# vribeiro1/artspeech

Measured on AMD Instinct MI355X. Metric: articulator-frames/sec (fwd+bwd), higher is better.
Workload: dtype f32

## Files before the change

### artspeech_amd/build.py

```python
import os
import subprocess
import sys

HERE = os.path.dirname(os.path.abspath(__file__))
ROOT = os.path.dirname(HERE)
CSRC = os.path.join(HERE, "csrc")
OBJ = os.path.join(HERE, "csrc", "build")
LIB = os.path.join(HERE, "libartspeech_hip.so")

ARCH = "gfx950"
COMMON = ["-O3", "-fPIC", "-std=c++17", f"-I{os.path.join(ROOT, 'include')}", f"-I{CSRC}"]
SOURCES = {
    "error.cpp": [],
    "prof.hip": [],
    "gemm_f32.hip": [],
    "wgrad_f32.hip": [],
    "lin_f32.hip": [],
    "gemm_s6.hip": [],
    "rowops.hip": [],
    "gru.hip": [],
    "lstm.hip": [],
    "conv.hip": [],
    "scorer_wgrad.hip": [],
    "ctc.hip": [],
    "recog_eval.hip": [],
    "attention.hip": [],
    "metrics.hip": ["-ffp-contract=off"],
    "p2cp_loss.hip": ["-ffp-contract=off"],
    "multi_mlp.hip": [],
    "pca.hip": [],
    "mean_contour.hip": [],
    "pc_eval.hip": ["-ffp-contract=off"],
    "report.hip": ["-ffp-contract=off"],
    "contours.hip": ["-ffp-contract=off"],
    "artspeech.hip": [],
}


def _newer(src, dst, extra=()):
    if not os.path.exists(dst):
        return True
    t = os.path.getmtime(dst)
    return any(os.path.getmtime(s) > t for s in (src, *extra))


def build(force=False, verbose=True):
    hipcc = os.environ.get("HIPCC", "/opt/rocm/bin/hipcc")
    os.makedirs(OBJ, exist_ok=True)
    headers = [os.path.join(CSRC, f) for f in os.listdir(CSRC) if f.endswith(".h")]
    headers.append(os.path.join(ROOT, "include", "artspeech_hip.h"))
    objs, relink = [], force
    for name, extra in SOURCES.items():
        src = os.path.join(CSRC, name)
        obj = os.path.join(OBJ, name.rsplit(".", 1)[0] + ".o")
        objs.append(obj)
        if force or _newer(src, obj, headers):
            cmd = [hipcc, f"--offload-arch={ARCH}", *COMMON, *extra, "-c", src, "-o", obj]
            if name.endswith(".cpp"):
                cmd = [hipcc, *COMMON, "-c", src, "-o", obj]
            if verbose:
                print("[build]", " ".join(cmd), flush=True)
            subprocess.check_call(cmd)
            relink = True
    if relink or not os.path.exists(LIB):
        cmd = [hipcc, f"--offload-arch={ARCH}", "-shared", "-fPIC", "-o", LIB, *objs]
        if verbose:
            print("[build]", " ".join(cmd), flush=True)
        subprocess.check_call(cmd)
    return LIB


if __name__ == "__main__":
    print(build(force="--force" in sys.argv))
```

### artspeech_amd/csrc/artspeech.hip

```cpp
#include <stdlib.h>

#include <algorithm>
#include <mutex>
#include <vector>

#include "as_launch.h"
#include "gemm_internal.h"
#include "rowops.h"

namespace {

constexpr int D = AS_HEAD_HIDDEN;
constexpr int64_t SLAB_FLOATS = 16LL << 20;
constexpr int64_t SLAB2_FLOATS = 28LL << 20;

struct Carve {
    int64_t off = 0;
    int64_t take(int64_t n) {
        const int64_t o = off;
        off += as_round_up(n, 64);
        return o;
    }
};

// ... 212 lines not shown
        lo.Bp = reinterpret_cast<const uint16_t*>(ws + w.w3p); lo.bp_rows = (int)as_round_up(O, OUT_BN);
        lo.bp_batch = as_planes_batch_stride(lo.bp_rows, D); lo.bp_plane = A * lo.bp_batch;
        int n_part = 0;
        if (crit) {
            lo.tgt = crit->tgt; lo.tgt_T = crit->tgt_T; lo.lengths = crit->lengths; lo.T = crit->T; lo.scale = crit->scale;
            lo.dout = crit->dout; lo.partial = ws + w.lpart; lo.partial_capacity = w.lpart_n; lo.loss = crit->loss;
        }
        took = as_lin_out_try(&lo, &n_part, st);
        AS_REQUIRE(took >= 0, took, "head gemm3: launch failed");
        if (took && crit && n_part > 0) AS_TRY(as_loss_final(ws + w.lpart, n_part, crit->scale, crit->loss, st));
        crit_done = took && crit;
        if (!took) {
            took = as_lin_try(&l3, st);
            AS_REQUIRE(took >= 0, took, "head gemm3: launch failed");
        }
    }
    if (!took)
        AS_STEP("head.gemm3", st, gemm_nt(ws + w.r2hat, AD, ws + w.w3f, D, out, (long)A * O, ws + w.b3f, R, O, D, 2, st, A, D,
                       (long)Opad * D, O, O));
    if (crit && !crit_done) {
        AS_STEP("loss", st, as_euclid_masked_fwd_bwd_presigmoid(out, crit->tgt, crit->tgt_T, crit->lengths, (int32_t)(rows / crit->T), crit->T, A,
                                                               d.n_samp, crit->scale, crit->loss, crit->dout, ws + w.lpart, st));
    }
    return 0;
}

int head_bwd_dx(const as_dims& d, const as_layout& L, const float* P, const float* out, const float* dout, int64_t rows,
                float* dx, const float* relu_src, float* ws, hipStream_t st, bool presig = false) {
    (void)L; (void)P;
    const int A = d.n_art, H = d.hidden, O = 2 * d.n_samp;
    const HeadWs w = head_ws(d, rows);
    const int R = (int)rows;
    const long AD = (long)A * D, AO = (long)A * O;
    const float* dpre3 = presig ? dout : ws + w.dpre3;
    if (!presig) AS_STEP("headb.sigmoid", st, as_sigmoid_bwd(out, dout, ws + w.dpre3, rows * AO, st));
    const int Opad = (int)as_round_up(O, 32);
    const unsigned long long* bits1 = reinterpret_cast<const unsigned long long*>(ws + w.bits1);
    const unsigned long long* bits2 = reinterpret_cast<const unsigned long long*>(ws + w.bits2);
    as_lin b3{};
    b3.A = dpre3; b3.lda = AO; b3.a_batch = O;
    b3.B = ws + w.w3f; b3.ldb = D; b3.b_batch = (long)Opad * D; b3.b_kc = 0;
    b3.C = ws + w.dz2; b3.ldc = AD; b3.c_batch = D;
    b3.M = R; b3.N = D; b3.K = Opad; b3.ka_valid = O; b3.batch = A; b3.epi = 2;
    b3.xhat = ws + w.r2hat; b3.ldx = AD; b3.x_batch = D; b3.rstd_in = ws + w.rstd2; b3.bits_in = bits2;
    b3.Bp = reinterpret_cast<const uint16_t*>(ws + w.w3tp); b3.bp_rows = D; b3.bp_batch = as_planes_batch_stride(D, Opad);
    b3.bp_plane = A * b3.bp_batch;
    int took;
    {
        AS_PROF("headb.dx3", st);
        took = as_lin_try(&b3, st);
        AS_REQUIRE(took >= 0, took, "head dx3: launch failed");
    }
    if (!took) {
        AS_STEP("headb.dx3", st, gemm_nn(dpre3, AO, ws + w.w3f, D, ws + w.dz2, AD, R, D, O, st, A, O, (long)Opad * D, D));
        AS_STEP("headb.norm2", st, as_normalize_bwd(ws + w.dz2, ws + w.r2hat, ws + w.rstd2, nullptr, ws + w.dz2, rows * A, D, st, bits2));
    }
    as_lin b2 = b3;
    b2.A = ws + w.dz2; b2.lda = AD; b2.a_batch = D;
    b2.B = ws + w.w2f; b2.b_batch = (long)D * D;
    b2.C = ws + w.dz1; b2.K = D; b2.ka_valid = D;
    b2.xhat = ws + w.r1hat; b2.rstd_in = ws + w.rstd1; b2.bits_in = bits1;
    b2.Bp = reinterpret_cast<const uint16_t*>(ws + w.w2tp); b2.bp_batch = as_planes_batch_stride(D, D); b2.bp_plane = A * b2.bp_batch;
    {
        AS_PROF("headb.dx2", st);
        took = as_lin_try(&b2, st);
        AS_REQUIRE(took >= 0, took, "head dx2: launch failed");
    }
    if (!took) {
        AS_STEP("headb.dx2", st, gemm_nn(ws + w.dz2, AD, ws + w.w2f, D, ws + w.dz1, AD, R, D, D, st, A, D, (long)D * D, D));
        AS_STEP("headb.norm1", st, as_normalize_bwd(ws + w.dz1, ws + w.r1hat, ws + w.rstd1, nullptr, ws + w.dz1, rows * A, D, st, bits1));
    }
    int dx1_slabs = 0;
    if (H <= 256 && H % 4 == 0) {
        as_lin l{};
        l.A = ws + w.dz1; l.lda = AD;
        l.Bp = reinterpret_cast<const uint16_t*>(ws + w.w1tp); l.bp_rows = (int)as_round_up(H, 128);
        l.bp_batch = as_planes_batch_stride(l.bp_rows, (int)AD); l.bp_plane = l.bp_batch;
        l.C = ws + w.slab; l.ldc = H;
        l.M = R; l.N = H; l.K = (int)AD; l.batch = 1;
        const int want = (int)std::max<int64_t>(1, std::min<int64_t>(8, 512 / std::max(1, as_cdiv(R, 64))));
        const int slabs = as_lin_plain_s6_slabs((int)AD, want);
        if ((int64_t)slabs * R * H <= SLAB_FLOATS) {
            AS_PROF("headb.dx1", st);
            const int took1 = as_lin_plain_s6(&l, want, (long)R * H, st);
            AS_REQUIRE(took1 >= 0, took1, "head dx1: launch failed");
            if (took1) dx1_slabs = slabs;
        }
    }
    if (!dx1_slabs)
        AS_STEP("headb.dx1", st, gemm_nn(ws + w.dz1, AD, ws + w.w1f, H, ws + w.dxhat, H, R, H, (int)AD, st, 1, 0, 0, 0, ws + w.slab));
    AS_STEP("headb.norm0", st, as_normalize_bwd(dx1_slabs ? ws + w.slab : ws + w.dxhat, ws + w.xhat, ws + w.rstd0, relu_src, dx, rows, H, st, nullptr,
                                                 dx1_slabs ? dx1_slabs : 1, (long)R * H));
    return 0;
}

struct TrunkJob { const float* dz; const float* y; float* dW; float* db; int H; };

int head_bwd_dw(const as_dims& d, const as_layout& L, const float* P, int64_t rows, float* G, float* ws, float* slab,
                hipStream_t st, const float* dpre3_in = nullptr, int cu_budget = 0, long slab_floats = SLAB_FLOATS,
                const TrunkJob* trunk = nullptr, int part = 0, int unfold_layers = -1) {
    const int A = d.n_art, H = d.hidden, O = 2 * d.n_samp;
    const HeadWs w = head_ws(d, rows);
    const int R = (int)rows;
    const long AD = (long)A * D, AO = (long)A * O;
    const float* dpre3 = dpre3_in ? dpre3_in : ws + w.dpre3;
    as_wgrad_job jobs[4] = {};
    as_gemm& g3 = jobs[0].g;
    g3.A = dpre3; g3.a_i = 1; g3.a_k = AO; g3.a_batch = O; g3.M = O;
    g3.B = ws + w.r2hat; g3.b_j = 1; g3.b_k = AD; g3.b_batch = D; g3.N = D;
    g3.C = ws + w.dw3f; g3.ldc = D; g3.c_batch = (long)O * D; g3.K = R; g3.batch = A;
    g3.colsum = G + L.b3; g3.colsum_batch = O;
    as_gemm& g1 = jobs[1].g;
    g1 = g3;
    g1.A = ws + w.xhat; g1.a_k = H; g1.a_batch = 0; g1.M = H;
    g1.B = ws + w.dz1;
    g1.C = ws + w.dw1f; g1.ldc = H; g1.c_batch = (long)D * H;
    g1.colsum = nullptr; g1.colsum_batch = 0;
    jobs[1].colsum_b = G + L.b1; jobs[1].colsum_b_batch = D; jobs[1].c_trans = 1;
    as_wgrad_job job2{};
    as_gemm& g2 = job2.g;
    g2 = g3;
    g2.A = ws + w.dz2; g2.a_k = AD; g2.a_batch = D; g2.M = D;
    g2.B = ws + w.r1hat;
    g2.C = ws + w.dw2f; g2.c_batch = (long)D * D;
    g2.colsum = G + L.b2; g2.colsum_batch = D;
    const bool multi_ok = R % 32 == 0 && R >= 512;
    if (part == 0 || part == 1) {
        int n = 2;
        const bool trunk_rides = trunk && 2 * trunk->H == 256;
        if (trunk_rides) {
            as_gemm& gt = jobs[n].g;
            gt.A = trunk->dz; gt.a_i = 1; gt.a_k = trunk->H; gt.M = trunk->H;
            gt.B = trunk->y; gt.b_j = 1; gt.b_k = 2 * trunk->H; gt.N = 2 * trunk->H;
            gt.C = trunk->dW; gt.ldc = 2 * trunk->H; gt.K = R; gt.batch = 1;
            gt.colsum = trunk->db; gt.colsum_batch = 0;
            ++n;
        }
        if (part == 0) jobs[n++] = job2;
        int took = 0;
        if (multi_ok) {
            AS_PROF(part == 0 ? "headb.dw_fused" : "headb.dw31", st);
            took = as_wgrad_multi(jobs, n, slab, slab_floats, cu_budget, st, cu_budget > 0);
            AS_REQUIRE(took >= 0, took, "head weight gradients: launch failed");
        }
        if (!took) {
            AS_STEP("headb.dw3", st, gemm_tn(dpre3, AO, ws + w.r2hat, AD, ws + w.dw3f, D, O, D, R, st, slab, G + L.b3, O, A, O, D, (long)O * D, 0, 0, 0, cu_budget));
            AS_STEP("headb.dw1", st, gemm_tn(ws + w.dz1, AD, ws + w.xhat, H, ws + w.dw1f, H, (int)AD, H, R, st, slab, G + L.b1, 0, 1, 0, 0, 0, 0, 0, 0, cu_budget));
            if (part == 0)
                AS_STEP("headb.dw2", st, gemm_tn(ws + w.dz2, AD, ws + w.r1hat, AD, ws + w.dw2f, D, D, D, R, st, slab, G + L.b2, D, A, D, D, (long)D * D, 0, 0, 0, cu_budget));
        }
        if (trunk && !(took && trunk_rides))
            AS_STEP("trunkb.dw", st, gemm_tn(trunk->dz, trunk->H, trunk->y, 2 * trunk->H, trunk->dW, 2 * trunk->H, trunk->H, 2 * trunk->H, R, st, slab, trunk->db, 0));
    } else {
        int took = 0;
        if (multi_ok) {
            AS_PROF("headb.dw2", st);
            took = as_wgrad_multi(&job2, 1, slab, slab_floats, cu_budget, st, cu_budget > 0);
            AS_REQUIRE(took >= 0, took, "head weight gradients: launch failed");
        }
        if (!took)
            AS_STEP("headb.dw2", st, gemm_tn(ws + w.dz2, AD, ws + w.r1hat, AD, ws + w.dw2f, D, D, D, R, st, slab, G + L.b2, D, A, D, D, (long)D * D, 0, 0, 0, cu_budget));
    }
    if (unfold_layers < 0) unfold_layers = part == 1 ? 0 : 7;
    if (unfold_layers == 0) return 0;
    const float* dWf[3]; const float* dbf[3]; const float* Wp[3]; const float* gm[3]; const float* bt[3];
    float* dWo[3]; float* dgm[3]; float* dbt[3];
    int Rs[3], Ks[3], cnt = 0;
// ... 379 lines not shown
```

### artspeech_amd/csrc/gemm_internal.h

```cpp
#pragma once
#include "as_common.h"

int as_wgrad_try(const as_gemm* g, hipStream_t st);
struct as_wgrad_job {
    as_gemm g;
    float* colsum_b; long colsum_b_batch;
    int c_trans;
};
int as_wgrad_multi(const as_wgrad_job* jobs, int n, float* slab, long slab_floats, int cu_budget, hipStream_t st, bool exact = false);

enum { AS_ARITH_FP32 = 0, AS_ARITH_BF16X6 = 1 };
int as_matrix_arith();

struct as_planes_job {
    const float* B; long n_stride, k_stride, batch_stride;
    int batch, N, K, rows_pad, Kpad;
    uint16_t* out;
};
int as_emit_planes(const as_planes_job* jobs, int n, hipStream_t st);
static inline long as_planes_batch_stride(int rows_pad, int Kpad) { return (long)(Kpad / 16) * rows_pad * 16; }
static inline long as_planes_floats(int batch, int rows_pad, int Kpad) { return 3 * batch * as_planes_batch_stride(rows_pad, Kpad) / 2; }

int as_gemm_s6_nt(const float* A, long lda, long a_batch, const float* B, long ldb, long b_batch, const float* bias, long bias_batch, float* C,
                  long ldc, long c_batch, int M, int N, int K, int batch, int act, hipStream_t st);
int as_gemm_s6_nt_ext(const as_gemm* g, hipStream_t st);
template <int N> struct IC2 { static constexpr int value = N; };

void as_stop_event_set_raw(void* ev);
void* as_stop_event_take_raw();
inline void as_stop_event_set(hipEvent_t ev) { as_stop_event_set_raw((void*)ev); }
inline hipEvent_t as_stop_event_take() { return (hipEvent_t)as_stop_event_take_raw(); }

struct as_lin {
    const float* A; long lda, a_batch;
    const float* B; long ldb, b_batch; int b_kc;
    const uint16_t* Bp; long bp_plane, bp_batch; int bp_rows;
    float* C; long ldc, c_batch;
    const float* bias; long bias_batch;
    int M, N, K, ka_valid, batch, act, epi;
    float* rstd; unsigned long long* bits;
    const float* xhat; long ldx, x_batch; const float* rstd_in; const unsigned long long* bits_in;
    int tile_rows;
};
int as_lin_try(const as_lin* a, hipStream_t st);
int as_lin_plain_s6(const as_lin* a, int ksplit, long c_split, hipStream_t st);
static inline int as_lin_plain_s6_slabs(int K, int ksplit) {
    if (ksplit < 1) ksplit = 1;
    const int kchunk = (int)as_round_up(as_cdiv(K, ksplit), 32);
    return as_cdiv(K, kchunk);
}

struct as_lin_out {
    const float* A; long lda, a_batch;
    const float* B; long ldb, b_batch; int b_rows;
    const float* bias; long bias_batch;
    float* out; long ldo, o_batch;
    int M, N, K, batch;
    const float* tgt; long tgt_T; const int* lengths; int T; float scale;
    float* dout; float* partial; long partial_capacity;
    const uint16_t* Bp; long bp_plane, bp_batch; int bp_rows;
    float* loss;
};
int as_lin_out_try(const as_lin_out* a, int* n_partials, hipStream_t st);
int* as_arrival_counter(hipStream_t st);
int as_loss_final(const float* partial, int n, float scale, float* loss, hipStream_t st);

bool as_gru_bwd_tokens_fits(int32_t V, int32_t H, int32_t T);
int as_gru_bidir_bwd_tokens(const float* dy, const float* y, const float* gates, const float* w_hh, const int32_t* lengths,
                            int32_t B, int32_t T, int32_t H, float* dgh, const int64_t* tokens, int64_t tok_stride, int32_t V,
                            float* part, hipStream_t st);
int as_gru_bidir_fwd_tokens(const float* table, const int64_t* tokens, int64_t tok_stride, int32_t V, const float* w_hh,
                            const float* b_hh, const int32_t* lengths, int32_t B, int32_t T, int32_t H, float* y, float* gates,
                            hipStream_t st);
int as_count_bad_tokens(const int64_t* tokens, long tok_stride, int T, long rows, int V, int* count, hipStream_t st);
int as_sum_partials(const float* part, long n, int chunks, float* out, hipStream_t st);
```

### artspeech_amd/csrc/lin_f32.hip

```cpp
#include <cstdlib>

#include <type_traits>

#include "gemm_internal.h"
#include "split_arith.h"

namespace {

constexpr int BN = 256, BK = 16, NT = 512, NBUF = 3;
enum { EPI_PLAIN = 0, EPI_LNF = 1, EPI_LNB = 2 };

struct LinK {
    const float* A; long lda, a_batch;
    const float* B; long ldb, b_batch;
    const uint16_t* Bp; long bp_plane, bp_batch; int bp_rows;
    int kchunk; long c_split;
    float* C; long ldc, c_batch;
    const float* bias; long bias_batch;
    int M, N, K, ka_valid, batch, act;
    int n_big, big_per_batch, big_per_batch_rows, small_per_batch;
    int tile_rows;
    unsigned long long* dbg; long dbg_max;
    float eps;
    float* rstd;
// ... 248 lines not shown
                __builtin_amdgcn_sched_barrier(0);
            }
        }
    };
    static_assert(BK == 16, "two fragment groups per k-tile");
    Frag f0, f1;
    load(f0, 0, 0);
    for (int kt = 0; kt < nk; ++kt) {
        load(f1, kt, 1);
        __builtin_amdgcn_sched_barrier(0);
        mma(f0, kt + AHEADT < nk ? kt + AHEADT : -1);
        __builtin_amdgcn_sched_barrier(0);
        if (kt + 2 < nk) asm volatile("s_waitcnt vmcnt(3)" ::: "memory");
        else asm volatile("s_waitcnt vmcnt(0)" ::: "memory");
        as_wait_lds();
        __builtin_amdgcn_s_barrier();
        if (kt + 1 < nk) load(f0, kt + 1, 0);
        __builtin_amdgcn_sched_barrier(0);
        mma(f1, -1);
        __builtin_amdgcn_sched_barrier(0);
    }
    if (stamp) g.dbg[8L * blockIdx.x + 2] = __builtin_amdgcn_s_memtime();

    lin_epilogue<TM, EPI>(g, acc, smem, bz, m0, tm_eff, wave, lane);
    if (stamp) {
        asm volatile("s_waitcnt vmcnt(0)" ::: "memory");
        g.dbg[8L * blockIdx.x + 3] = __builtin_amdgcn_s_memtime();
        g.dbg[8L * blockIdx.x + 6] = __builtin_amdgcn_s_memrealtime();
    }
}

__device__ __forceinline__ int xcd_contiguous(int b, int total) {
    const int q = total >> 3, r = total & 7, x = b & 7, i = b >> 3;
    return x * q + min(x, r) + i;
}

constexpr int S6_BK = 32;
constexpr int S6_PLANE = 64 * S6_BK * 2;
constexpr int S6_BUF = 3 * S6_PLANE;

template <int N> struct IC { static constexpr int value = N; };

template <int NW, int TME>
__device__ __forceinline__ void s6_main_loop(f32x16 (&acc)[2], unsigned char* sm, const float* __restrict__ A, long lda, int rows_valid,
                                             int K, int ka_valid, const uint16_t* __restrict__ bp, unsigned b_lane, long bp_plane,
                                             long bp_step, int tid, int lane, bool late, unsigned long long* stamp1 = nullptr) {
    constexpr int NTH = NW * 64;
    constexpr int AL = 512 / NTH;
    const int l31 = lane & 31, lh = lane >> 5;
    const int a_chunk = tid & 7;
    unsigned a_off[AL];
    int a_wr[AL];
#pragma unroll
    for (int q = 0; q < AL; ++q) {
        const int row = (tid >> 3) + q * (NTH / 8);
        a_off[q] = (unsigned)(min(row, rows_valid - 1) * (int)lda + a_chunk * 4) * 4u;
        a_wr[q] = row * 64 + (((a_chunk >> 1) ^ ((row >> 2) & 3)) * 16) + (a_chunk & 1) * 8;
    }
    const int nk = K / S6_BK, nj = 2 * nk;
    const gptr Au = as_uniform_ptr(A);
    auto a_load = [&](f32x4 (&dst)[AL], int kt) {
        kt = min(kt, nk - 1);
        const unsigned ko = kt * S6_BK + a_chunk * 4 + 4 <= ka_valid ? (unsigned)(kt * S6_BK) * 4u : 0u - (unsigned)a_chunk * 16u;
#pragma unroll
        for (int q = 0; q < AL; ++q) dst[q] = *reinterpret_cast<gptr_f4>(Au + (a_off[q] + ko));
    };
    auto a_store = [&](const f32x4 (&src)[AL], int buf) {
#pragma unroll
        for (int q = 0; q < AL; ++q) {
            unsigned h0, m0, l0, h1, m1, l1;
            split_pair(src[q].x, src[q].y, h0, m0, l0);
            split_pair(src[q].z, src[q].w, h1, m1, l1);
            unsigned char* d = sm + buf * S6_BUF + a_wr[q];
            *reinterpret_cast<uint2*>(d) = make_uint2(h0, h1);
            *reinterpret_cast<uint2*>(d + S6_PLANE) = make_uint2(m0, m1);
            *reinterpret_cast<uint2*>(d + 2 * S6_PLANE) = make_uint2(l0, l1);
        }
    };
    auto b_load = [&](u32x4 (&dst)[3], int j) {
        j = min(j, nj - 1);
#pragma unroll
        for (int p = 0; p < 3; ++p) dst[p] = *reinterpret_cast<gptr_u4>(as_uniform_ptr(bp + p * bp_plane + j * bp_step) + b_lane);
    };
    const int sw = (l31 >> 2) & 3;
    const unsigned char* a_rd = sm + l31 * 64;

    f32x4 aq[3][AL];
    u32x4 bq[3][3];
    a_load(aq[0], 0);
    a_load(aq[1], 1);
    b_load(bq[0], 0);
    b_load(bq[1], 1);
    a_store(aq[0], 0);
    as_lds_barrier();
    if (stamp1) *stamp1 = __builtin_amdgcn_s_memtime();
    auto tile = [&](auto Uc, int kt) {
        constexpr int U = decltype(Uc)::value;
        const unsigned char* img = a_rd + (kt & 1) * S6_BUF;
        a_load(aq[(U + 2) % 3], kt + 2);
#pragma unroll
        for (int s = 0; s < 2; ++s) {
            b_load(bq[(2 * U + s + 2) % 3], 2 * kt + s + 2);
            __builtin_amdgcn_sched_barrier(0);
            bf16x8 fa[TME][3];
#pragma unroll
            for (int p = 0; p < 3; ++p)
#pragma unroll
                for (int i = 0; i < TME; ++i)
                    fa[i][p] = *reinterpret_cast<const bf16x8*>(img + p * S6_PLANE + i * 32 * 64 + (((2 * s + lh) ^ sw) * 16));
            const u32x4(&bs)[3] = bq[(2 * U + s) % 3];
            bf16x8 fb[3];
#pragma unroll
            for (int p = 0; p < 3; ++p) fb[p] = __builtin_bit_cast(bf16x8, bs[p]);
            constexpr int PA[6] = {0, 0, 0, 1, 1, 2}, PB[6] = {0, 1, 2, 0, 1, 0};
#pragma unroll
            for (int o = 0; o < 6; ++o)
#pragma unroll
                for (int i = 0; i < TME; ++i)
                    acc[i] = __builtin_amdgcn_mfma_f32_32x32x16_bf16(fa[i][PA[o]], fb[PB[o]], acc[i], 0, 0, 0);
            __builtin_amdgcn_sched_barrier(0);
            if (late == (s == 0)) a_store(aq[(U + 1) % 3], (kt & 1) ^ 1);
        }
        as_lds_barrier();
    };
    int kt = 0;
    for (; kt + 3 <= nk; kt += 3) {
        tile(IC<0>{}, kt);
        tile(IC<1>{}, kt + 1);
        tile(IC<2>{}, kt + 2);
    }
    if (kt < nk) tile(IC<0>{}, kt);
    if (kt + 1 < nk) tile(IC<1>{}, kt + 1);
}

template <int EPI>
__global__ __launch_bounds__(NT, 4) void lin_s6_kernel(LinK g) {
    constexpr int EPIT = 32 * BN;
    static_assert(EPIT * 4 >= 2 * S6_BUF, "the epilogue's staging area holds both plane images");
    __shared__ __attribute__((aligned(16))) float smem[EPIT];
    int bz, m0, tm_eff;
    const int tile = blockIdx.x;
    if (tile < g.n_big) {
        bz = tile / g.big_per_batch;
        m0 = (tile - bz * g.big_per_batch) * 64;
        tm_eff = 2;
    } else {
        const int j = tile - g.n_big;
        bz = j / g.small_per_batch;
        m0 = g.big_per_batch_rows + (j - bz * g.small_per_batch) * 32;
        tm_eff = 1;
    }
    const int tid = threadIdx.x, lane = tid & 63, wave = tid >> 6;
    f32x16 acc[2];
#pragma unroll
    for (int i = 0; i < 2; ++i)
#pragma unroll
        for (int r = 0; r < 16; ++r) acc[i][r] = 0.f;
    const uint16_t* bp = g.Bp + (long)bz * g.bp_batch;
    const unsigned b_lane = (unsigned)((wave * 32 + (lane & 31)) * 16 + (lane >> 5) * 8) * 2u;
    unsigned char* sm = reinterpret_cast<unsigned char*>(smem);
    const float* A = g.A + (long)bz * g.a_batch + (long)m0 * g.lda;
    const bool late = __builtin_amdgcn_readfirstlane(wave) >= 4;
    const bool stamp = g.dbg != nullptr && tid == 0 && blockIdx.x < g.dbg_max;
    unsigned long long* d = stamp ? g.dbg + 8L * blockIdx.x : nullptr;
    if (stamp) {
        d[0] = __builtin_amdgcn_s_memtime();
        d[4] = __builtin_amdgcn_s_memrealtime();
        d[5] = __builtin_amdgcn_s_getreg((4 - 1) << 11 | 0 << 6 | 4) | ((unsigned long long)__builtin_amdgcn_s_getreg((32 - 1) << 11 | 0 << 6 | 20) << 32);
    }
    if (tm_eff == 2) s6_main_loop<8, 2>(acc, sm, A, g.lda, g.M - m0, g.K, g.ka_valid, bp, b_lane, g.bp_plane, (long)g.bp_rows * 16, tid, lane, late, stamp ? d + 1 : nullptr);
    else s6_main_loop<8, 1>(acc, sm, A, g.lda, g.M - m0, g.K, g.ka_valid, bp, b_lane, g.bp_plane, (long)g.bp_rows * 16, tid, lane, late, stamp ? d + 1 : nullptr);
    if (stamp) d[2] = __builtin_amdgcn_s_memtime();
    lin_epilogue<2, EPI>(g, acc, smem, bz, m0, tm_eff, wave, lane);
    if (stamp) {
        asm volatile("s_waitcnt vmcnt(0)" ::: "memory");
        d[3] = __builtin_amdgcn_s_memtime();
        d[6] = __builtin_amdgcn_s_memrealtime();
    }
}

template <int NW>
__global__ __launch_bounds__(NW * 64, 4) void lin_s6_plain_kernel(LinK g) {
    __shared__ __attribute__((aligned(16))) unsigned char sm[2 * S6_BUF];
    int bz, m0, tm_eff;
    const int tile = blockIdx.x;
    if (tile < g.n_big) {
        bz = tile / g.big_per_batch;
        m0 = (tile - bz * g.big_per_batch) * 64;
        tm_eff = 2;
    } else {
        const int j = tile - g.n_big;
        bz = j / g.small_per_batch;
        m0 = g.big_per_batch_rows + (j - bz * g.small_per_batch) * 32;
        tm_eff = 1;
    }
    const int tid = threadIdx.x, lane = tid & 63, wave = tid >> 6;
    const int l31 = lane & 31, lh = lane >> 5;
    const int ks = blockIdx.y, k0 = ks * g.kchunk;
    const int klen = min(g.kchunk, g.K - k0);
    const int kav = max(0, min(klen, g.ka_valid - k0));
    f32x16 acc[2];
#pragma unroll
    for (int i = 0; i < 2; ++i)
#pragma unroll
        for (int r = 0; r < 16; ++r) acc[i][r] = 0.f;
    const long bp_step = (long)g.bp_rows * 16;
    const uint16_t* bp = g.Bp + (long)bz * g.bp_batch + (k0 / 16) * bp_step;
    const unsigned b_lane = (unsigned)((wave * 32 + l31) * 16 + lh * 8) * 2u;
    const float* A = g.A + (long)bz * g.a_batch + (long)m0 * g.lda + k0;
    const bool late = __builtin_amdgcn_readfirstlane(wave) >= NW / 2;
    if (tm_eff == 2) s6_main_loop<NW, 2>(acc, sm, A, g.lda, g.M - m0, klen, kav, bp, b_lane, g.bp_plane, bp_step, tid, lane, late);
    else s6_main_loop<NW, 1>(acc, sm, A, g.lda, g.M - m0, klen, kav, bp, b_lane, g.bp_plane, bp_step, tid, lane, late);
    const int col = wave * 32 + l31;
    if (col >= g.N) return;
    const bool whole = gridDim.y == 1;
    const float bj = (whole && g.bias) ? g.bias[(long)bz * g.bias_batch + col] : 0.f;
    float* c0 = g.C + (long)ks * g.c_split + (long)bz * g.c_batch + col;
#pragma unroll
    for (int i = 0; i < 2; ++i)
#pragma unroll
        for (int r = 0; r < 16; ++r) {
            const int row = m0 + i * 32 + (r & 3) + 8 * (r >> 2) + 4 * lh;
            if (i < tm_eff && row < g.M) {
                float v = acc[i][r] + bj;
                if (whole && g.act == 1) v = as_relu(v);
                else if (whole && g.act == 2) v = as_sigmoid(v);
                c0[(long)row * g.ldc] = v;
            }
        }
}

constexpr int ON = 128;

struct LinOutK {
    const float* A; long lda, a_batch;
    const float* B; long ldb, b_batch; int b_rows;
    const float* bias; long bias_batch;
    float* out; long ldo, o_batch;
    int M, N, K, batch;
    int n_big, big_per_batch, big_per_batch_rows, small_per_batch;
    const float* tgt; long tgt_T; const int* lengths; int T; float scale;
    float* dout; float* partial;
    const uint16_t* Bp; long bp_plane, bp_batch; int bp_rows;
    float* loss; int* counter;
};

__device__ __forceinline__ void criterion_tail(const LinOutK& g, int tile, float sum, int tid, float* red, int nwaves) {
    if (g.counter == nullptr) {
        if (tid == 0) g.partial[tile] = sum;
        return;
    }
    __shared__ int s_last;
    if (tid == 0) {
        __hip_atomic_store(&g.partial[tile], sum, __ATOMIC_RELAXED, __HIP_MEMORY_SCOPE_AGENT);
        asm volatile("s_waitcnt vmcnt(0)" ::: "memory");
        const int last = atomicAdd(g.counter, 1) == (int)gridDim.x - 1;
        if (last) __hip_atomic_store(g.counter, 0, __ATOMIC_RELAXED, __HIP_MEMORY_SCOPE_AGENT);
        s_last = last;
    }
    __syncthreads();
    if (!s_last) return;
    float s = 0.f;
    if (tid < 256)
        for (int i = tid; i < (int)gridDim.x; i += 256) s += __hip_atomic_load(&g.partial[i], __ATOMIC_RELAXED, __HIP_MEMORY_SCOPE_AGENT);
    s = as_wave_sum(s);
    __syncthreads();
    if ((tid & 63) == 0 && tid < 256) red[tid >> 6] = s;
    __syncthreads();
    if (tid == 0) g.loss[0] = ((red[0] + red[1]) + (red[2] + red[3])) * g.scale;
    (void)nwaves;
}

__global__ __launch_bounds__(NT, 4) void lin_out_kernel(LinOutK g) {
    constexpr int TILE = BK * (64 + ON);
    constexpr int RING = NBUF * TILE;
    __shared__ __attribute__((aligned(16))) float smem[RING];
    int bz, m0, rows;
    if ((int)blockIdx.x < g.n_big) {
// ... 73 lines not shown
    if (active) {
#pragma unroll
        for (int r = 0; r < 16; ++r) smem[(wm * 32 + (r & 3) + 8 * (r >> 2) + 4 * lh) * ON + col] = as_sigmoid(acc[r] + bj);
    }
    as_lds_barrier();
    const int Np = g.N >> 1;
    float part = 0.f;
    const int wave_u = __builtin_amdgcn_readfirstlane(wave);
    if (Np <= 64) {
        float tx[8], ty[8];
        bool in[8], valid[8];
        const int nl = min(lane, Np - 1);
#pragma unroll
        for (int k = 0; k < 8; ++k) {
            const int r = wave_u + 8 * k;
            const int frame = m0 + r;
            in[k] = r < rows && frame < g.M;
            const int fc = in[k] ? frame : m0;
            const int b = fc / g.T, t = fc - b * g.T;
            valid[k] = in[k] && t < g.lengths[b];
            const float* tg = g.tgt + (((long)b * g.tgt_T + t) * g.batch + bz) * g.N;
            tx[k] = tg[nl];
            ty[k] = tg[Np + nl];
        }
#pragma unroll
        for (int k = 0; k < 8; ++k) {
            if (!in[k]) continue;
            const int r = wave_u + 8 * k;
            const long frame = m0 + r;
            float* o = g.out + frame * g.ldo + (long)bz * g.o_batch;
            float* dz = g.dout + frame * g.ldo + (long)bz * g.o_batch;
            if (lane < Np) {
                const float ox = smem[r * ON + lane], oy = smem[r * ON + Np + lane];
                o[lane] = ox;
                o[Np + lane] = oy;
                float gx = 0.f, gy = 0.f;
                if (valid[k]) {
                    const float dx = ox - tx[k], dy = oy - ty[k];
                    const float d = sqrtf(dx * dx + dy * dy);
                    part += d;
                    const float gg = g.scale / d;
                    gx = dx * gg * ox * (1.f - ox);
                    gy = dy * gg * oy * (1.f - oy);
                }
                dz[lane] = gx;
                dz[Np + lane] = gy;
            }
        }
    } else
    for (int r = wave_u; r < rows; r += 8) {
        const int frame = m0 + r;
        if (frame >= g.M) break;
        const int b = frame / g.T, t = frame - b * g.T;
        const bool valid = t < g.lengths[b];
        float* o = g.out + (long)frame * g.ldo + (long)bz * g.o_batch;
        float* dz = g.dout + (long)frame * g.ldo + (long)bz * g.o_batch;
        const float* tg = g.tgt + (((long)b * g.tgt_T + t) * g.batch + bz) * g.N;
        for (int n = lane; n < Np; n += 64) {
            const float ox = smem[r * ON + n], oy = smem[r * ON + Np + n];
            o[n] = ox;
            o[Np + n] = oy;
            float gx = 0.f, gy = 0.f;
            if (valid) {
                const float dx = ox - tg[n], dy = oy - tg[Np + n];
                const float d = sqrtf(dx * dx + dy * dy);
                part += d;
                const float gg = g.scale / d;
                gx = dx * gg * ox * (1.f - ox);
                gy = dy * gg * oy * (1.f - oy);
            }
            dz[n] = gx;
            dz[Np + n] = gy;
        }
    }
    part = as_wave_sum_dpp(part);
    __shared__ float red[8];
    if (lane == 0) red[wave] = part;
    __syncthreads();
    float wg_sum = 0.f;
    if (tid == 0) wg_sum = ((red[0] + red[1]) + (red[2] + red[3])) + ((red[4] + red[5]) + (red[6] + red[7]));
    criterion_tail(g, blockIdx.x, wg_sum, tid, red, 8);
}

__global__ __launch_bounds__(256, 4) void lin_out_s6_kernel(LinOutK g) {
    __shared__ __attribute__((aligned(16))) float smem[64 * ON];
    static_assert(64 * ON * 4 >= 2 * S6_BUF, "the epilogue's tile holds both plane images");
    int bz, m0, rows;
    const int tile = blockIdx.x;
    if (tile < g.n_big) {
        bz = tile / g.big_per_batch;
        m0 = (tile - bz * g.big_per_batch) * 64;
        rows = 64;
    } else {
        const int j = tile - g.n_big;
        bz = j / g.small_per_batch;
        m0 = g.big_per_batch_rows + (j - bz * g.small_per_batch) * 32;
        rows = 32;
    }
    const int tid = threadIdx.x, lane = tid & 63, wave = tid >> 6;
    const int l31 = lane & 31, lh = lane >> 5;
    f32x16 acc[2];
#pragma unroll
    for (int i = 0; i < 2; ++i)
#pragma unroll
        for (int r = 0; r < 16; ++r) acc[i][r] = 0.f;
    const uint16_t* bp = g.Bp + (long)bz * g.bp_batch;
    const unsigned b_lane = (unsigned)((wave * 32 + l31) * 16 + lh * 8) * 2u;
    unsigned char* sm = reinterpret_cast<unsigned char*>(smem);
    const float* A = g.A + (long)bz * g.a_batch + (long)m0 * g.lda;
    const int wave_u = __builtin_amdgcn_readfirstlane(wave);
    if (rows == 64) s6_main_loop<4, 2>(acc, sm, A, g.lda, g.M - m0, g.K, g.K, bp, b_lane, g.bp_plane, (long)g.bp_rows * 16, tid, lane, wave_u >= 2);
    else s6_main_loop<4, 1>(acc, sm, A, g.lda, g.M - m0, g.K, g.K, bp, b_lane, g.bp_plane, (long)g.bp_rows * 16, tid, lane, wave_u >= 2);
    const int col = wave * 32 + l31;
    const float bj = (g.bias && col < g.N) ? g.bias[(long)bz * g.bias_batch + col] : 0.f;
    const int nblk = rows / 32;
    if (g.tgt == nullptr) {
        if (col < g.N) {
            float* o0 = g.out + (long)bz * g.o_batch + col;
#pragma unroll
            for (int i = 0; i < 2; ++i)
#pragma unroll
                for (int r = 0; r < 16; ++r) {
                    const int row = m0 + i * 32 + (r & 3) + 8 * (r >> 2) + 4 * lh;
                    if (i < nblk && row < g.M) o0[(long)row * g.ldo] = as_sigmoid(acc[i][r] + bj);
                }
        }
        return;
    }
#pragma unroll
    for (int i = 0; i < 2; ++i)
#pragma unroll
        for (int r = 0; r < 16; ++r)
            if (i < nblk) smem[(i * 32 + (r & 3) + 8 * (r >> 2) + 4 * lh) * ON + col] = as_sigmoid(acc[i][r] + bj);
    as_lds_barrier();
    const int Np = g.N >> 1;
    float part = 0.f;
    if (Np <= 64) {
        const int nl = min(lane, Np - 1);
        float tx[16], ty[16];
        bool in[16], valid[16];
#pragma unroll
        for (int k = 0; k < 16; ++k) {
            const int r = wave_u + 4 * k;
            const int frame = m0 + r;
            in[k] = r < rows && frame < g.M;
            const int fc = in[k] ? frame : m0;
            const int b = fc / g.T, t = fc - b * g.T;
            valid[k] = in[k] && t < g.lengths[b];
            const float* tg = g.tgt + (((long)b * g.tgt_T + t) * g.batch + bz) * g.N;
            tx[k] = tg[nl];
            ty[k] = tg[Np + nl];
        }
#pragma unroll
        for (int k = 0; k < 16; ++k) {
            if (!in[k]) continue;
            const int r = wave_u + 4 * k;
            const long frame = m0 + r;
            float* o = g.out + frame * g.ldo + (long)bz * g.o_batch;
            float* dz = g.dout + frame * g.ldo + (long)bz * g.o_batch;
            if (lane < Np) {
                const float ox = smem[r * ON + lane], oy = smem[r * ON + Np + lane];
                o[lane] = ox;
                o[Np + lane] = oy;
                float gx = 0.f, gy = 0.f;
                if (valid[k]) {
                    const float dx = ox - tx[k], dy = oy - ty[k];
                    const float d = sqrtf(dx * dx + dy * dy);
                    part += d;
                    const float gg = g.scale / d;
                    gx = dx * gg * ox * (1.f - ox);
                    gy = dy * gg * oy * (1.f - oy);
                }
                dz[lane] = gx;
                dz[Np + lane] = gy;
            }
        }
    } else
    for (int r = wave_u; r < rows; r += 4) {
        const int frame = m0 + r;
        if (frame >= g.M) break;
        const int b = frame / g.T, t = frame - b * g.T;
// ... 20 lines not shown
    }
    part = as_wave_sum_dpp(part);
    __shared__ float red[4];
    if (lane == 0) red[wave] = part;
    __syncthreads();
    float wg_sum = 0.f;
    if (tid == 0) wg_sum = (red[0] + red[1]) + (red[2] + red[3]);
    criterion_tail(g, tile, wg_sum, tid, red, 4);
}

inline bool aligned16(const void* p) { return (reinterpret_cast<uintptr_t>(p) & 15) == 0; }

template <bool B_KC, int EPI>
int launch(const LinK& k, hipStream_t st) {
    LinK kk = k;
    constexpr int slots = 512;
    const long units = (long)as_cdiv(k.M, 64) * k.batch;
    const long rounds = units / slots;
    int x = (int)(rounds * slots / k.batch);
    if (x > k.M / 64 || k.tile_rows == 64) x = k.M / 64;
    if (k.tile_rows == 32) x = 0;
    const int rest = k.M - x * 64;
    kk.big_per_batch = x > 0 ? x : 1;
    kk.big_per_batch_rows = x * 64;
    kk.n_big = x * k.batch;
    kk.small_per_batch = as_cdiv(rest, 32);
    const long total = (long)kk.n_big + (long)kk.small_per_batch * k.batch;
    if (kk.small_per_batch == 0) kk.small_per_batch = 1;
    if (kk.Bp) {
        hipLaunchKernelGGL((lin_s6_kernel<EPI>), dim3((unsigned)total), dim3(NT), 0, st, kk);
        AS_LAUNCH_CHECK("as_lin_s6");
        return 0;
    }
    hipLaunchKernelGGL((lin_f32_kernel<64, B_KC, EPI>), dim3((unsigned)total), dim3(NT), 0, st, kk);
    AS_LAUNCH_CHECK("as_lin_f32");
    return 0;
}

unsigned long long* g_dbg = nullptr;
long g_dbg_max = 0;

}

extern "C" void as_lin_debug_stamps(uint64_t* buf, int64_t max_workgroups) {
    g_dbg = (unsigned long long*)buf;
    g_dbg_max = buf ? max_workgroups : 0;
}

int as_lin_try(const as_lin* a, hipStream_t st) {
    if (a->K % BK || a->K < BK || a->N > BN || a->N < 4 || a->M < 1 || a->batch < 1) return 0;
    if (!aligned16(a->A) || !aligned16(a->B) || a->lda % 4 || a->ldb % 4 || a->a_batch % 4 || a->b_batch % 4) return 0;
    if (!a->b_kc && a->N % 4) return 0;
    if (a->epi != EPI_PLAIN && (a->N != BN || !a->C)) return 0;
    if (a->epi == EPI_PLAIN && a->N <= BN / 2) return 0;
    if ((long)as_cdiv(a->M, 64) * a->batch > (1L << 30)) return 0;
    LinK k{};
    k.A = a->A; k.lda = a->lda; k.a_batch = a->a_batch;
    k.B = a->B; k.ldb = a->ldb; k.b_batch = a->b_batch;
    k.C = a->C; k.ldc = a->ldc; k.c_batch = a->c_batch;
    k.bias = a->bias; k.bias_batch = a->bias_batch;
    k.M = a->M; k.N = a->N; k.K = a->K; k.ka_valid = a->ka_valid > 0 ? a->ka_valid : a->K; k.batch = a->batch; k.act = a->act;
    k.tile_rows = a->tile_rows;
    k.eps = 1e-5f;
    k.dbg = g_dbg; k.dbg_max = g_dbg_max;
    k.rstd = a->rstd; k.bits = a->bits;
    k.xhat = a->xhat; k.ldx = a->ldx; k.x_batch = a->x_batch; k.rstd_in = a->rstd_in; k.bits_in = a->bits_in;
    if (k.ka_valid % 4) return 0;
    if (a->Bp && as_matrix_arith() == AS_ARITH_BF16X6 && a->K % S6_BK == 0 && a->bp_rows >= BN && (reinterpret_cast<uintptr_t>(a->Bp) & 15) == 0 &&
        a->bp_plane % 8 == 0 && a->bp_batch % 8 == 0 && a->lda < (1L << 23)) {
        k.Bp = a->Bp; k.bp_plane = a->bp_plane; k.bp_batch = a->bp_batch; k.bp_rows = a->bp_rows;
    }
    if (a->epi == EPI_LNF) {
        if (!a->rstd || !a->bits || !a->b_kc) return 0;
        return launch<true, EPI_LNF>(k, st) == 0 ? 1 : -1;
    }
    if (a->epi == EPI_LNB) {
        if (!a->xhat || !a->rstd_in || !a->bits_in || a->b_kc) return 0;
        return launch<false, EPI_LNB>(k, st) == 0 ? 1 : -1;
    }
    if (a->b_kc) return launch<true, EPI_PLAIN>(k, st) == 0 ? 1 : -1;
    return launch<false, EPI_PLAIN>(k, st) == 0 ? 1 : -1;
}

int as_lin_plain_s6(const as_lin* a, int ksplit, long c_split, hipStream_t st) {
    if (as_matrix_arith() != AS_ARITH_BF16X6 || !a->Bp) return 0;
    if (a->epi != EPI_PLAIN || a->K % S6_BK || a->K < S6_BK || a->N > BN || a->N < 1 || a->M < 1 || a->batch < 1 || !a->C) return 0;
    if (!aligned16(a->A) || a->lda % 4 || a->a_batch % 4 || a->lda >= (1L << 23)) return 0;
    if ((reinterpret_cast<uintptr_t>(a->Bp) & 15) || a->bp_plane % 8 || a->bp_batch % 8) return 0;
    const int nw = a->N <= 128 ? 4 : 8;
    if (a->bp_rows < nw * 32) return 0;
    if (ksplit < 1) ksplit = 1;
    if (ksplit > 1 && (a->bias || a->act)) return 0;
    LinK k{};
    k.A = a->A; k.lda = a->lda; k.a_batch = a->a_batch;
    k.Bp = a->Bp; k.bp_plane = a->bp_plane; k.bp_batch = a->bp_batch; k.bp_rows = a->bp_rows;
    k.C = a->C; k.ldc = a->ldc; k.c_batch = a->c_batch;
    k.bias = a->bias; k.bias_batch = a->bias_batch;
    k.M = a->M; k.N = a->N; k.K = a->K; k.ka_valid = a->ka_valid > 0 ? a->ka_valid : a->K; k.batch = a->batch; k.act = a->act;
    if (k.ka_valid % 4) return 0;
    k.kchunk = (int)as_round_up(as_cdiv(a->K, ksplit), S6_BK);
    ksplit = as_cdiv(a->K, k.kchunk);
    k.c_split = c_split;
    int tile = a->tile_rows;
    if (tile != 32 && tile != 64) tile = (long)as_cdiv(a->M, 64) * a->batch * ksplit >= 384 ? 64 : 32;
    const int x = tile == 64 ? a->M / 64 : 0;
    const int rest = a->M - x * 64;
    k.big_per_batch = x > 0 ? x : 1;
    k.big_per_batch_rows = x * 64;
    k.n_big = x * a->batch;
    k.small_per_batch = as_cdiv(rest, 32);
    const long total = (long)k.n_big + (long)k.small_per_batch * a->batch;
    if (k.small_per_batch == 0) k.small_per_batch = 1;
    if (total > (1L << 30) || ksplit > 65535) return 0;
    if (nw == 4) hipLaunchKernelGGL((lin_s6_plain_kernel<4>), dim3((unsigned)total, ksplit), dim3(256), 0, st, k);
    else hipLaunchKernelGGL((lin_s6_plain_kernel<8>), dim3((unsigned)total, ksplit), dim3(512), 0, st, k);
    AS_LAUNCH_CHECK("as_lin_plain_s6");
    return 1;
}

int as_lin_out_try(const as_lin_out* a, int* n_partials, hipStream_t st) {
    if (a->K % BK || a->K < BK || a->N > ON || a->N < 4 || a->N % 2 || a->M < 1 || a->batch < 1) return 0;
    if (!aligned16(a->A) || !aligned16(a->B) || a->lda % 4 || a->ldb % 4 || a->a_batch % 4 || a->b_batch % 4) return 0;
    if (a->b_rows < a->N) return 0;
    LinOutK k{};
    k.A = a->A; k.lda = a->lda; k.a_batch = a->a_batch;
    k.B = a->B; k.ldb = a->ldb; k.b_batch = a->b_batch; k.b_rows = a->b_rows;
    k.bias = a->bias; k.bias_batch = a->bias_batch;
    k.out = a->out; k.ldo = a->ldo; k.o_batch = a->o_batch;
    k.M = a->M; k.N = a->N; k.K = a->K; k.batch = a->batch;
    k.tgt = a->tgt; k.tgt_T = a->tgt_T; k.lengths = a->lengths; k.T = a->T; k.scale = a->scale; k.dout = a->dout; k.partial = a->partial;
    if (k.tgt && (!k.lengths || !k.dout || !k.partial || k.T < 1 || k.ldo != (long)k.batch * k.N || k.o_batch != k.N)) return 0;
    constexpr int slots = 1024;
    const long units = (long)as_cdiv(k.M, 64) * k.batch;
    const long rounds = units / slots;
    int x = (int)(rounds * slots / k.batch);
    if (x > k.M / 64) x = k.M / 64;
    if (rounds == 0) x = k.M / 64;
    const int rest = k.M - x * 64;
    k.big_per_batch = x > 0 ? x : 1;
    k.big_per_batch_rows = x * 64;
    k.n_big = x * k.batch;
    k.small_per_batch = as_cdiv(rest, 32);
    const long total = (long)k.n_big + (long)k.small_per_batch * k.batch;
    if (k.small_per_batch == 0) k.small_per_batch = 1;
    if (k.tgt && total > a->partial_capacity) return 0;
    if (k.tgt && a->loss) {
        k.counter = as_arrival_counter(st);
        k.loss = k.counter ? a->loss : nullptr;
    }
    const int left = k.counter ? 0 : (int)total;
    if (a->Bp && as_matrix_arith() == AS_ARITH_BF16X6 && a->K % S6_BK == 0 && a->bp_rows >= ON && (reinterpret_cast<uintptr_t>(a->Bp) & 15) == 0 &&
        a->bp_plane % 8 == 0 && a->bp_batch % 8 == 0 && a->lda < (1L << 23)) {
        k.Bp = a->Bp; k.bp_plane = a->bp_plane; k.bp_batch = a->bp_batch; k.bp_rows = a->bp_rows;
        hipLaunchKernelGGL(lin_out_s6_kernel, dim3((unsigned)total), dim3(256), 0, st, k);
        AS_LAUNCH_CHECK("as_lin_out_s6");
        if (n_partials) *n_partials = left;
        return 1;
    }
    hipLaunchKernelGGL(lin_out_kernel, dim3((unsigned)total), dim3(NT), 0, st, k);
    AS_LAUNCH_CHECK("as_lin_out");
    if (n_partials) *n_partials = left;
    return 1;
}

namespace {
inline bool linear_blocks(int N, int* bn, int* nb) {
    if (N <= 256) { *bn = N <= 128 ? 128 : 256; *nb = 1; return true; }
    if (N % 256 == 0) { *bn = 256; *nb = N / 256; return true; }
    return false;
}
}

extern "C" int64_t as_linear_planes_floats(int32_t N, int32_t K) {
    int bn, nb;
    if (N < 1 || K < 1 || !linear_blocks(N, &bn, &nb)) return 0;
    return as_round_up(as_planes_floats(nb, bn, (int)as_round_up(K, 32)), 64);
}

extern "C" int as_linear_fwd(const float* A, int64_t lda, const float* W, int64_t ldw, const float* bias, float* out, int64_t ldo,
                             int32_t M, int32_t N, int32_t K, int32_t act, float* planes_ws, void* stream) {
    AS_REQUIRE(A && W && out && M > 0 && N > 0 && K > 0 && lda >= K && ldw >= K && ldo >= N && act >= 0 && act <= 2, AS_ERR_BAD_ARG,
               "as_linear_fwd: bad argument");
    hipStream_t st = (hipStream_t)stream;
    int bn, nb;
    if (!planes_ws) {
        const int took = as_gemm_s6_nt(A, lda, 0, W, ldw, 0, bias, 0, out, ldo, 0, M, N, K, 1, act, st);
        AS_REQUIRE(took >= 0, took, "as_linear_fwd: launch failed");
        if (took) return 0;
    }
    if (as_matrix_arith() == AS_ARITH_BF16X6 && planes_ws && K % S6_BK == 0 && lda % 4 == 0 && linear_blocks(N, &bn, &nb) &&
        (reinterpret_cast<uintptr_t>(planes_ws) & 15) == 0) {
        const int rows_last = N - (nb - 1) * bn;
        as_planes_job j{W, ldw, 1, (long)bn * ldw, nb, nb > 1 ? bn : rows_last, K, bn, K, reinterpret_cast<uint16_t*>(planes_ws)};
        AS_TRY(as_emit_planes(&j, 1, st));
        as_lin l{};
        l.A = A; l.lda = lda;
        l.Bp = reinterpret_cast<const uint16_t*>(planes_ws); l.bp_rows = bn; l.bp_batch = as_planes_batch_stride(bn, K); l.bp_plane = nb * l.bp_batch;
        l.C = out; l.ldc = ldo; l.c_batch = bn;
// ... 12 lines not shown
```

Baseline: 6.263 million.

## Tune register pressure and occupancy bounds for bf16x6 linear kernels

Adds a waves-per-SIMD template parameter to the plain s6 linear kernel and uses 2 for the head dx1 backward GEMM, lowers the min-occupancy bound of lin_out_s6_kernel from 4 to 3, and makes block-uniform indices scalar via readfirstlane. It also recomputes the LDS read swizzle and lane-derived offsets after the main loop behind an asm barrier, so those values need not stay live in registers across it. The build now captures kernel resource-usage remarks into per-file text files. The aim is to relieve register pressure and spills, accepting lower occupancy in exchange.

Result: faster. 6.401 million (median of 6 runs) (+2.2%).

```diff
diff --git a/artspeech_amd/build.py b/artspeech_amd/build.py
--- a/artspeech_amd/build.py
+++ b/artspeech_amd/build.py
@@ -1,4 +1,5 @@
 import os
+import re
 import subprocess
 import sys
 
@@ -44,6 +45,39 @@
     return any(os.path.getmtime(s) > t for s in (src, *extra))
 
 
+def resources_path(name):
+    return os.path.join(OBJ, name.rsplit(".", 1)[0] + ".resources.txt")
+
+
+def compile_one(name, extra, obj, hipcc, verbose=True):
+    src = os.path.join(CSRC, name)
+    if name.endswith(".cpp"):
+        cmd = [hipcc, *COMMON, "-c", src, "-o", obj]
+        if verbose:
+            print("[build]", " ".join(cmd), flush=True)
+        subprocess.check_call(cmd)
+        return
+    cmd = [hipcc, f"--offload-arch={ARCH}", *COMMON, *extra, "-Rpass-analysis=kernel-resource-usage", "-c", src, "-o", obj]
+    if verbose:
+        print("[build]", " ".join(cmd), flush=True)
+    r = subprocess.run(cmd, stderr=subprocess.PIPE, text=True)
+    remarks, rest, quoted = [], [], False
+    for line in r.stderr.splitlines(keepends=True):
+        if "[-Rpass-analysis=kernel-resource-usage]" in line:
+            remarks.append(line)
+            quoted = True
+        elif quoted and re.match(r"\s+\d*\s*\|", line):
+            continue
+        else:
+            rest.append(line)
+            quoted = False
+    sys.stderr.write("".join(rest))
+    if r.returncode:
+        raise subprocess.CalledProcessError(r.returncode, cmd)
+    with open(resources_path(name), "w") as f:
+        f.writelines(remarks)
+
+
 def build(force=False, verbose=True):
     hipcc = os.environ.get("HIPCC", "/opt/rocm/bin/hipcc")
     os.makedirs(OBJ, exist_ok=True)
@@ -55,12 +89,7 @@
         obj = os.path.join(OBJ, name.rsplit(".", 1)[0] + ".o")
         objs.append(obj)
         if force or _newer(src, obj, headers):
-            cmd = [hipcc, f"--offload-arch={ARCH}", *COMMON, *extra, "-c", src, "-o", obj]
-            if name.endswith(".cpp"):
-                cmd = [hipcc, *COMMON, "-c", src, "-o", obj]
-            if verbose:
-                print("[build]", " ".join(cmd), flush=True)
-            subprocess.check_call(cmd)
+            compile_one(name, extra, obj, hipcc, verbose)
             relink = True
     if relink or not os.path.exists(LIB):
         cmd = [hipcc, f"--offload-arch={ARCH}", "-shared", "-fPIC", "-o", LIB, *objs]
diff --git a/artspeech_amd/csrc/artspeech.hip b/artspeech_amd/csrc/artspeech.hip
--- a/artspeech_amd/csrc/artspeech.hip
+++ b/artspeech_amd/csrc/artspeech.hip
@@ -318,7 +318,7 @@
         const int slabs = as_lin_plain_s6_slabs((int)AD, want);
         if ((int64_t)slabs * R * H <= SLAB_FLOATS) {
             AS_PROF("headb.dx1", st);
-            const int took1 = as_lin_plain_s6(&l, want, (long)R * H, st);
+            const int took1 = as_lin_plain_s6(&l, want, (long)R * H, st, 2);
             AS_REQUIRE(took1 >= 0, took1, "head dx1: launch failed");
             if (took1) dx1_slabs = slabs;
         }
diff --git a/artspeech_amd/csrc/gemm_internal.h b/artspeech_amd/csrc/gemm_internal.h
--- a/artspeech_amd/csrc/gemm_internal.h
+++ b/artspeech_amd/csrc/gemm_internal.h
@@ -43,7 +43,7 @@
     int tile_rows;
 };
 int as_lin_try(const as_lin* a, hipStream_t st);
-int as_lin_plain_s6(const as_lin* a, int ksplit, long c_split, hipStream_t st);
+int as_lin_plain_s6(const as_lin* a, int ksplit, long c_split, hipStream_t st, int waves_per_simd = 4);
 static inline int as_lin_plain_s6_slabs(int K, int ksplit) {
     if (ksplit < 1) ksplit = 1;
     const int kchunk = (int)as_round_up(as_cdiv(K, ksplit), 32);
diff --git a/artspeech_amd/csrc/lin_f32.hip b/artspeech_amd/csrc/lin_f32.hip
--- a/artspeech_amd/csrc/lin_f32.hip
+++ b/artspeech_amd/csrc/lin_f32.hip
@@ -354,8 +354,9 @@
 #pragma unroll
         for (int p = 0; p < 3; ++p) dst[p] = *reinterpret_cast<gptr_u4>(as_uniform_ptr(bp + p * bp_plane + j * bp_step) + b_lane);
     };
-    const int sw = (l31 >> 2) & 3;
+    int sw = (l31 >> 2) & 3;
     const unsigned char* a_rd = sm + l31 * 64;
+    int lh_rd = lh;
 
     f32x4 aq[3][AL];
     u32x4 bq[3][3];
@@ -379,7 +380,7 @@
             for (int p = 0; p < 3; ++p)
 #pragma unroll
                 for (int i = 0; i < TME; ++i)
-                    fa[i][p] = *reinterpret_cast<const bf16x8*>(img + p * S6_PLANE + i * 32 * 64 + (((2 * s + lh) ^ sw) * 16));
+                    fa[i][p] = *reinterpret_cast<const bf16x8*>(img + p * S6_PLANE + i * 32 * 64 + (((2 * s + lh_rd) ^ sw) * 16));
             const u32x4(&bs)[3] = bq[(2 * U + s) % 3];
             bf16x8 fb[3];
 #pragma unroll
@@ -400,6 +401,13 @@
         tile(IC<0>{}, kt);
         tile(IC<1>{}, kt + 1);
         tile(IC<2>{}, kt + 2);
+    }
+    {
+        int ln = lane;
+        asm volatile("" : "+v"(ln));
+        lh_rd = ln >> 5;
+        sw = ((ln & 31) >> 2) & 3;
+        a_rd = sm + (ln & 31) * 64;
     }
     if (kt < nk) tile(IC<0>{}, kt);
     if (kt + 1 < nk) tile(IC<1>{}, kt + 1);
@@ -422,6 +430,8 @@
         m0 = g.big_per_batch_rows + (j - bz * g.small_per_batch) * 32;
         tm_eff = 1;
     }
+    bz = __builtin_amdgcn_readfirstlane(bz);
+    m0 = __builtin_amdgcn_readfirstlane(m0);
     const int tid = threadIdx.x, lane = tid & 63, wave = tid >> 6;
     f32x16 acc[2];
 #pragma unroll
@@ -451,8 +461,8 @@
     }
 }
 
-template <int NW>
-__global__ __launch_bounds__(NW * 64, 4) void lin_s6_plain_kernel(LinK g) {
+template <int NW, int WPS>
+__global__ __launch_bounds__(NW * 64, WPS) void lin_s6_plain_kernel(LinK g) {
     __shared__ __attribute__((aligned(16))) unsigned char sm[2 * S6_BUF];
     int bz, m0, tm_eff;
     const int tile = blockIdx.x;
@@ -466,6 +476,8 @@
         m0 = g.big_per_batch_rows + (j - bz * g.small_per_batch) * 32;
         tm_eff = 1;
     }
+    bz = __builtin_amdgcn_readfirstlane(bz);
+    m0 = __builtin_amdgcn_readfirstlane(m0);
     const int tid = threadIdx.x, lane = tid & 63, wave = tid >> 6;
     const int l31 = lane & 31, lh = lane >> 5;
     const int ks = blockIdx.y, k0 = ks * g.kchunk;
@@ -705,7 +717,8 @@
     criterion_tail(g, blockIdx.x, wg_sum, tid, red, 8);
 }
 
-__global__ __launch_bounds__(256, 4) void lin_out_s6_kernel(LinOutK g) {
+constexpr int LOUT_WPS = 3;
+__global__ __launch_bounds__(256, LOUT_WPS) void lin_out_s6_kernel(LinOutK g) {
     __shared__ __attribute__((aligned(16))) float smem[64 * ON];
     static_assert(64 * ON * 4 >= 2 * S6_BUF, "the epilogue's tile holds both plane images");
     int bz, m0, rows;
@@ -720,6 +733,8 @@
         m0 = g.big_per_batch_rows + (j - bz * g.small_per_batch) * 32;
         rows = 32;
     }
+    bz = __builtin_amdgcn_readfirstlane(bz);
+    m0 = __builtin_amdgcn_readfirstlane(m0);
     const int tid = threadIdx.x, lane = tid & 63, wave = tid >> 6;
     const int l31 = lane & 31, lh = lane >> 5;
     f32x16 acc[2];
@@ -906,7 +921,7 @@
     return launch<false, EPI_PLAIN>(k, st) == 0 ? 1 : -1;
 }
 
-int as_lin_plain_s6(const as_lin* a, int ksplit, long c_split, hipStream_t st) {
+int as_lin_plain_s6(const as_lin* a, int ksplit, long c_split, hipStream_t st, int waves_per_simd) {
     if (as_matrix_arith() != AS_ARITH_BF16X6 || !a->Bp) return 0;
     if (a->epi != EPI_PLAIN || a->K % S6_BK || a->K < S6_BK || a->N > BN || a->N < 1 || a->M < 1 || a->batch < 1 || !a->C) return 0;
     if (!aligned16(a->A) || a->lda % 4 || a->a_batch % 4 || a->lda >= (1L << 23)) return 0;
@@ -936,8 +951,9 @@
     const long total = (long)k.n_big + (long)k.small_per_batch * a->batch;
     if (k.small_per_batch == 0) k.small_per_batch = 1;
     if (total > (1L << 30) || ksplit > 65535) return 0;
-    if (nw == 4) hipLaunchKernelGGL((lin_s6_plain_kernel<4>), dim3((unsigned)total, ksplit), dim3(256), 0, st, k);
-    else hipLaunchKernelGGL((lin_s6_plain_kernel<8>), dim3((unsigned)total, ksplit), dim3(512), 0, st, k);
+    if (nw == 4 && waves_per_simd == 2) hipLaunchKernelGGL((lin_s6_plain_kernel<4, 2>), dim3((unsigned)total, ksplit), dim3(256), 0, st, k);
+    else if (nw == 4) hipLaunchKernelGGL((lin_s6_plain_kernel<4, 4>), dim3((unsigned)total, ksplit), dim3(256), 0, st, k);
+    else hipLaunchKernelGGL((lin_s6_plain_kernel<8, 4>), dim3((unsigned)total, ksplit), dim3(512), 0, st, k);
     AS_LAUNCH_CHECK("as_lin_plain_s6");
     return 1;
 }
```
